# craftsangjae/instance-segmentation-road-project

Measured on AMD Instinct MI355X. Metric: images/sec at 1024x1024 (MaskLab inference hot path, full forward), higher is better.
Workload: dtype f32; 1 GPU; resnext50_full_b8_1024; per_gpu_batch=8, global_batch=8, height=1024, width=1024, parallelism=dp1, hipgraph=False, inputs=resident in HBM, weights=random init (cls logits x8 so NMS / mask head run at full load)

## Files before the change

### include/masklab_hip.h

```cpp
#ifndef MASKLAB_HIP_H
#define MASKLAB_HIP_H

#include <stdint.h>

#ifdef __cplusplus
extern "C" {
#endif

#define ML_OK 0
#define ML_E_BADARG (-1)
#define ML_E_LAUNCH (-2)
#define ML_E_NOGPU  (-3)

enum { ML_ACT_NONE = 0, ML_ACT_RELU = 1, ML_ACT_RELU6 = 2, ML_ACT_SIGMOID = 3 };
enum { ML_MATH_F32 = 0, ML_MATH_F16 = 1, ML_MATH_F16S = 2, ML_MATH_F32X3 = 3 };

#define ML_ABI_VERSION 7
int ml_version(void);
const char *ml_last_error(void);
int ml_device_check(void);

typedef struct ml_conv2d_desc {
    const float *in;
    const float *wgt;
// ... 185 lines not shown
    const void *residual;
    const float *w1, *b1;
    const float *w2, *b2;
    void *out;
    int32_t B, HW, C, Hd;
} ml_se_bottleneck_desc;
int64_t ml_se_bottleneck_workspace_bytes(int32_t B, int32_t HW, int32_t C);
int ml_se_bottleneck_f32(const ml_se_bottleneck_desc *desc, void *workspace, int64_t workspace_bytes, void *stream);
int ml_se_bottleneck_f16(const ml_se_bottleneck_desc *desc, void *workspace, int64_t workspace_bytes, void *stream);

int ml_conv1x1_dual_f32(const float *a, const float *x, const float *wgt, const float *bias, float *out,
                        int32_t B, int32_t H, int32_t W, int32_t Ka, int32_t Kx, int32_t N, int32_t stride, void *stream);
int ml_conv1x1_dual_f16(const void *a, const void *x, const void *wgt, const float *bias, void *out,
                        int32_t B, int32_t H, int32_t W, int32_t Ka, int32_t Kx, int32_t N, int32_t stride, void *stream);

int ml_restore_boxes_f32(const float *loc, const int32_t *priors, float *boxes,
                         int32_t B, int32_t A, void *stream);

int64_t ml_detection_workspace_bytes(int32_t B, int32_t A, int32_t C, int32_t max_out);
int ml_detection_proposal_f32(const float *cls_pred, const float *boxes, float *proposed,
                              int32_t *counts, int32_t *kept, float *gather_payload,
                              int32_t B, int32_t A, int32_t C,
                              float min_confidence, float nms_iou, float post_iou, int32_t max_out,
                              void *workspace, void *stream);

int ml_mask_distribute_i32(const float *rows, int32_t row_stride, int32_t has_k,
                           float *kvals , int32_t *level_slots,
                           int32_t *level_counts, int32_t *level_max, int32_t B, int32_t cap,
                           int32_t max_k, float base_size, void *stream);

// ... 215 lines not shown
```

### instance-segmentation-road-project_amd/csrc/conv1x1_pipe.hip

```cpp
#include <type_traits>
#include "common.h"

namespace {

constexpr int BM = 128, BN = 128;
constexpr int ROWB = 128;
constexpr int BUFB = (BM + BN) * ROWB;
constexpr int SCR_LD = 36;
constexpr int SCRB = 16 * SCR_LD * 4;
constexpr int pipe_lds_bytes(int nstage) { return nstage * BUFB + 4 * SCRB; }
constexpr int PIPE_MAX_NBG = 8;

struct f32x3_t { float v; };

typedef int i32x4 __attribute__((ext_vector_type(4)));
typedef unsigned u32x4 __attribute__((ext_vector_type(4)));

struct PipeArgs {
    const void *in, *wgt, *res;
    const float *bias;
    void *out;
    long long M;
    int K, N;
    int in_cs, in_coff, out_cs, out_coff;
    int panels, NB, grid;
    int units, gshift, NBG;
    int xcd_map;
    float lo, hi;
};

__device__ __forceinline__ void lds_dma16(__amdgpu_buffer_rsrc_t rsrc, char *dst, int voff, int soff) {
#if defined(__HIP_DEVICE_COMPILE__)
    __builtin_amdgcn_raw_ptr_buffer_load_lds(rsrc, (__attribute__((address_space(3))) void *)dst, 16, voff, soff, 0, 0);
#endif
}
__device__ __forceinline__ void buf_store16(f32x4 v, __amdgpu_buffer_rsrc_t rsrc, int voff, int soff) {
#if defined(__HIP_DEVICE_COMPILE__)
    __builtin_amdgcn_raw_buffer_store_b128(__builtin_bit_cast(u32x4, v), rsrc, voff, soff, 0);
#endif
}

__device__ __forceinline__ unsigned records_left(long long off, long long total) {
    const unsigned long long left = (unsigned long long)(total - off);
    const unsigned hi = (unsigned)(left >> 32), lo = (unsigned)left;
    return (hi & 0x80000000u) ? 0u : (hi ? 0xffffffffu : lo);
// ... 79 lines not shown
            v1[c] = __builtin_amdgcn_fmed3f(v1[c], S.lo, S.hi);
        }
    }
    if constexpr (F32) {
        buf_store16(v0, ro, S.t_voff[qn], S.rowoff[(qm * 2 + hs) * 2 + 0]);
        buf_store16(v1, ro, S.t_voff[qn], S.rowoff[(qm * 2 + hs) * 2 + 1]);
    } else {
        const f16x8 o = {(_Float16)v0[0], (_Float16)v0[1], (_Float16)v0[2], (_Float16)v0[3],
                         (_Float16)v1[0], (_Float16)v1[1], (_Float16)v1[2], (_Float16)v1[3]};
        buf_store16(__builtin_bit_cast(f32x4, o), ro, S.t_voff[qn], S.rowoff[(qm * 2 + hs) * 2]);
    }
}

template <class T, bool FIRST, bool HAS_RES, int NB4, bool CLAMP>
__device__ __forceinline__ void pipe_chunk(f32x16 (&cur)[2][2], f32x16 (&oth)[2][2], const PipeState &S, const char *rd,
                                           char *wr, char *scratch, __amdgpu_buffer_rsrc_t ra_nx,
                                           __amdgpu_buffer_rsrc_t rb_nx, int soff_nx, __amdgpu_buffer_rsrc_t ro_prev,
                                           const f32x4 (&bias_prev)[2][NB4], i32x4 rr_prev) {
    constexpr bool F32 = std::is_same<T, float>::value;
    constexpr int NSLOT = F32 ? 64 : 16;
    constexpr int UNITS = F32 ? 2 : 1;
    constexpr int LEAD = HAS_RES ? RES_LEAD : 0;
    constexpr int NREG = FIRST ? NPC + LEAD : 0;
    f32x4 ring[RES_LEAD][2];
    f32x4 fa[2][2], fb[2][2];
    auto read_frags = [&](int ks, f32x4 (&a)[2], f32x4 (&b)[2]) {
#pragma unroll
        for (int m = 0; m < 2; ++m)
            a[m] = *reinterpret_cast<const f32x4 *>(rd + S.a_off + m * 32 * ROWB + (((ks * 2 + S.h) ^ S.swz) * 16));
#pragma unroll
        for (int n = 0; n < 2; ++n)
            b[n] = *reinterpret_cast<const f32x4 *>(rd + S.b_off + n * 32 * ROWB + (((ks * 2 + S.h) ^ S.swz) * 16));
// ... 7 lines not shown
        f32x4 (&a)[2] = fa[ks & 1];
        f32x4 (&b)[2] = fb[ks & 1];
        if constexpr (in_ks == (F32 ? 6 : 1) && ks < 3) read_frags(ks + 1, fa[(ks + 1) & 1], fb[(ks + 1) & 1]);
        constexpr bool start = FIRST && ks == 0 && j == 0;
        const f32x16 zero = {0.f, 0.f, 0.f, 0.f, 0.f, 0.f, 0.f, 0.f, 0.f, 0.f, 0.f, 0.f, 0.f, 0.f, 0.f, 0.f};
        if constexpr (F32) {
            if constexpr (start) cur[mi][ni] = __builtin_amdgcn_mfma_f32_32x32x2f32(a[mi][j], b[ni][j], zero, 0, 0, 0);
            else cur[mi][ni] = __builtin_amdgcn_mfma_f32_32x32x2f32(a[mi][j], b[ni][j], cur[mi][ni], 0, 0, 0);
        } else {
            const f16x8 ha = __builtin_bit_cast(f16x8, a[mi]), hb = __builtin_bit_cast(f16x8, b[ni]);
            if constexpr (start) cur[mi][ni] = __builtin_amdgcn_mfma_f32_32x32x16_f16(ha, hb, zero, 0, 0, 0);
            else cur[mi][ni] = __builtin_amdgcn_mfma_f32_32x32x16_f16(ha, hb, cur[mi][ni], 0, 0, 0);
        }
        __builtin_amdgcn_sched_barrier(0);
        if constexpr (idx < 4) {
            lds_dma16(ra_nx, wr + (32 * idx + 8 * S.wave_u) * ROWB, S.a_voff[idx], soff_nx);
        } else if constexpr (idx < 8) {
            lds_dma16(rb_nx, wr + (BM + 32 * (idx - 4) + 8 * S.wave_u) * ROWB, S.b_voff[idx - 4], soff_nx);
        } else if constexpr (FIRST) {
            constexpr int pb = ((idx - 8) * NREG) / (NSLOT - 8), pe = ((idx - 7) * NREG) / (NSLOT - 8);
            static_for<pb, pe>([&](auto pc) {
                constexpr int p = decltype(pc)::value;
                if constexpr (p >= LEAD) {
                    constexpr int q = p - LEAD;
                    if constexpr (HAS_RES) {
                        constexpr int loads_after = ((p < NPC ? p : NPC) - q - 1) * UNITS;
                        constexpr int stores_after = (q - (q >= LEAD ? q - LEAD + 1 : 0)) * UNITS;
                        constexpr int younger = loads_after + stores_after;
                        static_assert(younger >= 0 && younger <= 63, "vmcnt immediate out of range");
                        if constexpr (F32) wait_loaded<younger>(ring[q % RES_LEAD][0], ring[q % RES_LEAD][1]);
                        else wait_loaded<younger>(ring[q % RES_LEAD][0]);
// ... 89 lines not shown
                for (int ni = 0; ni < 2; ++ni) cur[mi][ni] = __builtin_amdgcn_mfma_f32_32x32x16_f16(ah[mi], bh[ni], cur[mi][ni], 0, 0, 0);
#pragma unroll
            for (int mi = 0; mi < 2; ++mi)
#pragma unroll
                for (int ni = 0; ni < 2; ++ni) crx[mi][ni] = __builtin_amdgcn_mfma_f32_32x32x16_f16(ah[mi], bl[ni], crx[mi][ni], 0, 0, 0);
        }
#pragma unroll
        for (int mi = 0; mi < 2; ++mi)
#pragma unroll
            for (int ni = 0; ni < 2; ++ni)
                crx[mi][ni] = __builtin_amdgcn_mfma_f32_32x32x16_f16(al[mi], bh[ni], crx[mi][ni], 0, 0, 0);
        __builtin_amdgcn_sched_barrier(0);
    }
}

template <class T, bool HAS_RES, int NSTAGE, bool CLAMP>
__global__ void __launch_bounds__(256, NSTAGE == 2 ? 2 : 1)
conv1x1_pipe_kernel(const PipeArgs A) {
    constexpr bool X3 = std::is_same<T, f32x3_t>::value;
    constexpr bool F32 = !std::is_same<T, _Float16>::value;
    constexpr int ES = sizeof(T);
    constexpr int KC = ROWB / ES;
    constexpr int NB4 = F32 ? 1 : 2;
    extern __shared__ __align__(16) char lds[];
    const int tid = threadIdx.x, lane = tid & 63, wave = tid >> 6;
    const int wm = wave >> 1, wn = wave & 1;
    const int r = lane & 31, h = lane >> 5;
    const int ld_row = tid >> 3;
    const int ld_g = (tid & 7) ^ ((ld_row >> 1) & 7);

    PipeState S;
    S.h = h;
    S.swz = (r >> 1) & 7;
    S.a_off = (wm * 64 + r) * ROWB;
    S.b_off = BM * ROWB + (wn * 64 + r) * ROWB;
    S.wave_u = __builtin_amdgcn_readfirstlane(wave);
    S.lo = A.lo;
    S.hi = A.hi;
#pragma unroll
    for (int i = 0; i < 4; ++i) {
        S.a_voff[i] = ((ld_row + 32 * i) * A.in_cs + A.in_coff) * ES + ld_g * 16;
        S.b_voff[i] = (ld_row + 32 * i) * A.K * ES + ld_g * 16;
    }
    const int t_row = F32 ? (lane >> 3) : (lane >> 2);
    const int t_col = F32 ? (lane & 7) * 4 : (lane & 3) * 8;
#pragma unroll
    for (int ni = 0; ni < 2; ++ni)
        S.t_voff[ni] = ((wm * 64 + t_row) * A.out_cs + A.out_coff + wn * 64 + ni * 32 + t_col) * ES;
#pragma unroll
    for (int mi = 0; mi < 2; ++mi)
#pragma unroll
        for (int hs = 0; hs < 2; ++hs)
#pragma unroll
            for (int i = 0; i < 2; ++i) S.rowoff[(mi * 2 + hs) * 2 + i] = (mi * 32 + hs * 16 + 8 * i) * A.out_cs * ES;
    S.scr_w = (4 * h * SCR_LD + r) * 4;
    S.scr_r = (t_row * SCR_LD + t_col) * 4;

    const int nk = A.K / KC;
    const long long in_total = A.M * (long long)A.in_cs * ES;
    const long long out_total = A.M * (long long)A.out_cs * ES;
    const long long w_total = (long long)A.N * A.K * ES;
    const int gmask = (1 << A.gshift) - 1;
    const int step = A.grid >> A.gshift;
    const int bid = (int)blockIdx.x;
    const int slot = bid >> 3, ppx = step >> 3;
    const int group = A.xcd_map ? (slot & gmask) : (bid & gmask);
    const int panel0 = A.xcd_map ? (bid & 7) * ppx + (slot >> A.gshift) : (bid >> A.gshift);
    auto panel_of = [&](Cursor c) { return c.u; };
    auto res_a = [&](Cursor c) { return rsrc_at(A.in, (long long)panel_of(c) * BM * A.in_cs * ES, c.u < A.panels ? in_total : 0); };
    auto res_b = [&](Cursor c) { return rsrc_at(A.wgt, (long long)c.nt * BN * A.K * ES, c.u < A.panels ? w_total : 0); };
    auto tile_off = [&](Cursor c) { return ((long long)panel_of(c) * BM * A.out_cs + (long long)c.nt * BN) * ES; };
    auto res_o = [&](Cursor c) { return rsrc_at(A.out, tile_off(c), c.u < A.panels ? out_total : 0); };
    auto res_words = [&](Cursor c) { return rsrc_words(A.res, tile_off(c), (HAS_RES && c.u < A.panels) ? out_total : 0); };
    const int nt0 = group * A.NBG;
    auto advance = [&](Cursor c) {
        Cursor n = c;
        if (n.nt + 1 < nt0 + A.NBG) { ++n.nt; } else { n.u += step; n.nt = nt0; }
        return n;
    };
    char *scratch = lds + NSTAGE * BUFB + S.wave_u * SCRB;
    float *lds_bias = reinterpret_cast<float *>(lds + NSTAGE * BUFB + 4 * SCRB);
    for (int i = tid; i < A.NBG * BN; i += 256) lds_bias[i] = A.bias ? A.bias[nt0 * BN + i] : 0.f;
    __syncthreads();
    auto bias_at = [&](Cursor c) { return lds_bias + (c.u < A.panels ? c.nt - nt0 : 0) * BN + wn * 64 + t_col; };
// ... 10 lines not shown
    if (cur.u >= A.panels) return;
    Cursor nx = cur;
    int kc_nx = 0;

    f32x16 accA[2][2], accB[2][2];
    f32x4 bias_cur[2][NB4], bias_prev[2][NB4];
#pragma unroll
    for (int ni = 0; ni < 2; ++ni)
#pragma unroll
        for (int k = 0; k < NB4; ++k) bias_prev[ni][k] = f32x4{0.f, 0.f, 0.f, 0.f};
    load_bias(cur, bias_cur);
#pragma unroll
    for (int st = 0; st < NSTAGE - 1; ++st) {
        const __amdgpu_buffer_rsrc_t ra = res_a(nx), rb = res_b(nx);
        const int soff = kc_nx * ROWB;
#pragma unroll
        for (int i = 0; i < 4; ++i) lds_dma16(ra, lds + st * BUFB + (32 * i + 8 * S.wave_u) * ROWB, S.a_voff[i], soff);
#pragma unroll
        for (int i = 0; i < 4; ++i) lds_dma16(rb, lds + st * BUFB + (BM + 32 * i + 8 * S.wave_u) * ROWB, S.b_voff[i], soff);
        ++kc_nx;
        if (kc_nx == nk) { kc_nx = 0; nx = advance(nx); }
    }
    asm volatile("s_waitcnt vmcnt(%0)" ::"n"(8 * (NSTAGE - 2)) : "memory");
    __builtin_amdgcn_s_barrier();

    Cursor prev = {A.panels, 0};
    int buf = 0;
    auto run_tile_x3 = [&](f32x16 (&acc)[2][2], f32x16 (&crx)[2][2]) -> bool {
        const Cursor next = advance(cur);
        const bool has_next = next.u < A.panels;
// ... 19 lines not shown
        prev = cur;
        cur = next;
        return has_next;
    };
    auto run_tile = [&](f32x16 (&acc)[2][2], f32x16 (&oth)[2][2]) -> bool {
        const Cursor next = advance(cur);
        const bool has_next = next.u < A.panels;
        const __amdgpu_buffer_rsrc_t ro_prev = res_o(prev);
        const i32x4 rr_prev = res_words(prev);
        for (int kc = 0; kc < nk; ++kc) {
            const __amdgpu_buffer_rsrc_t ra_nx = res_a(nx), rb_nx = res_b(nx);
            const int soff_nx = kc_nx * ROWB;
            const char *rd = lds + buf * BUFB;
            char *wr = lds + (buf == 0 ? NSTAGE - 1 : buf - 1) * BUFB;
            const bool first = kc == 0;
            if (first) pipe_chunk<T, true, HAS_RES, NB4, CLAMP>(acc, oth, S, rd, wr, scratch, ra_nx, rb_nx, soff_nx, ro_prev, bias_prev, rr_prev);
            else pipe_chunk<T, false, HAS_RES, NB4, CLAMP>(acc, oth, S, rd, wr, scratch, ra_nx, rb_nx, soff_nx, ro_prev, bias_prev, rr_prev);
            ++kc_nx;
            if (kc_nx == nk) { kc_nx = 0; nx = advance(nx); }
            buf = buf + 1 == NSTAGE ? 0 : buf + 1;
            if (kc <= NSTAGE - 2) asm volatile("s_waitcnt vmcnt(%0)" ::"n"(8 * (NSTAGE - 2) + (F32 ? 16 : 8)) : "memory");
            else asm volatile("s_waitcnt vmcnt(%0)" ::"n"(8 * (NSTAGE - 2)) : "memory");
            __builtin_amdgcn_s_barrier();
        }
        prev = cur;
#pragma unroll
        for (int ni = 0; ni < 2; ++ni)
#pragma unroll
            for (int k = 0; k < NB4; ++k) bias_prev[ni][k] = bias_cur[ni][k];
        cur = next;
        if (has_next) load_bias(cur, bias_cur);
        return has_next;
// ... 16 lines not shown
            }
            finish_piece<T, q, HAS_RES, NB4, CLAMP>(acc, S, scratch, ro, bias_prev, r0, r1);
        });
    };
    if constexpr (X3) {
        while (run_tile_x3(accA, accB)) {}
        x3_finish<HAS_RES, CLAMP>(accA, accB, S, scratch, res_o(prev), bias_at(prev), res_words(prev));
    } else {
        for (;;) {
            if (!run_tile(accA, accB)) { drain(accA); break; }
            if (!run_tile(accB, accA)) { drain(accB); break; }
        }
    }
}

template <class T, bool HAS_RES, int NSTAGE, bool CLAMP>
int launch_pipe(const PipeArgs &A, hipStream_t s) {
    auto kern = conv1x1_pipe_kernel<T, HAS_RES, NSTAGE, CLAMP>;
    static std::atomic<unsigned long long> ok{0};
    if (int rc = ml_ensure_dynamic_lds(reinterpret_cast<const void *>(kern), pipe_lds_bytes(NSTAGE) + 4 * PIPE_MAX_NBG * BN, ok,
                                       "conv1x1_pipe"))
        return rc;
    hipLaunchKernelGGL(kern, dim3(A.grid), dim3(256), pipe_lds_bytes(NSTAGE) + 4 * A.NBG * BN, s, A);
    ML_CHECK_LAUNCH("conv1x1_pipe");
    return ML_OK;
}

}

int ml_conv1x1_pipe_eligible(const ml_conv2d_desc &d) {
    const bool f16s = d.math == ML_MATH_F16S, x3 = d.math == ML_MATH_F32X3;
    const int kc = f16s ? 64 : 32;
    const bool shape_ok = d.KH == 1 && d.KW == 1 && d.stride == 1 && d.dil == 1 && d.pad_t == 0 && d.pad_l == 0 &&
                          d.cpp_shift == 30 && d.group_cin_step == 0 && d.shuffle2x2 == 0 && d.out_bstride == 0 &&
                          (d.math == ML_MATH_F32 || f16s || x3) && d.Ho == d.H && d.Wo == d.W;
    if (!shape_ok || d.live || d.gn_partials) return 0;
    if (f16s && !d.out_f16) return 0;
    if (!f16s && d.out_f16) return 0;
    if (d.span % kc != 0 || d.cout % 128 != 0 || d.n_pad != d.cout) return 0;
    if (!f16s && d.span != d.span_pad) return 0;
// ... 7 lines not shown
    int nbg = d.cout / BN;
    for (int g = 1; g < 8 && nbg > PIPE_MAX_NBG && nbg % 2 == 0 && (1 << g) <= ml_resident_blocks(2); ++g) nbg /= 2;
    return nbg <= PIPE_MAX_NBG;
}

int ml_conv1x1_pipe_try(const ml_conv2d_desc &d, hipStream_t s, int *eligible) {
    *eligible = 0;
    if (!ml_conv1x1_pipe_eligible(d)) return ML_OK;
    const long long M = (long long)d.B * d.H * d.W;
    PipeArgs A;
    A.in = d.in; A.wgt = d.wgt; A.bias = d.bias; A.res = d.residual; A.out = d.out;
    A.M = M; A.K = d.span; A.N = d.cout;
    A.in_cs = d.in_cstride; A.in_coff = d.in_coff; A.out_cs = d.out_cstride; A.out_coff = d.out_coff;
    A.panels = (int)((M + BM - 1) / BM);
    A.NB = d.cout / BN;
    const int resident = ml_resident_blocks(2);
    double eff_of[8] = {0, 0, 0, 0, 0, 0, 0, 0}, best_eff = -1.0;
    int n_g = 0;
    for (int g = 0; g < 8 && (A.NB >> g) >= 1 && (A.NB % (1 << g)) == 0; ++g) {
        n_g = g + 1;
        if ((A.NB >> g) > PIPE_MAX_NBG || (1 << g) > resident) continue;
        const long long units = (long long)A.panels << g;
        const long long grid = units < resident ? units : resident / (1 << g) * (1 << g);
        const long long rounds = (units + grid - 1) / grid;
        eff_of[g] = (double)units / (double)(rounds * resident);
        if (eff_of[g] > best_eff) best_eff = eff_of[g];
    }
    if (best_eff <= 0.0) return ML_OK;
    int best = -1, best_map = 0;
    for (int g = n_g - 1; g > 0 && best < 0; --g) {
        if (eff_of[g] <= 0.0 || eff_of[g] < best_eff - 0.02) continue;
        const long long units = (long long)A.panels << g;
        const long long grid = units < resident ? units : resident / (1 << g) * (1 << g);
        if (grid % (8ll << g) == 0) { best = g; best_map = 1; }
    }
    for (int g = 0; g < n_g && best < 0; ++g)
        if (eff_of[g] > 0.0 && eff_of[g] >= best_eff - 0.02) best = g;
    A.gshift = best;
    A.xcd_map = best_map;
    A.NBG = A.NB >> A.gshift;
    A.units = A.panels << A.gshift;
    A.grid = A.units < resident ? A.units : resident / (1 << A.gshift) * (1 << A.gshift);
    const bool clamp = d.act != ML_ACT_NONE;
    A.lo = 0.f;
    A.hi = d.act == ML_ACT_RELU6 ? 6.f : 3.402823466e38f;
    int rc;
    if (d.math == ML_MATH_F16S) {
        if (clamp) rc = d.residual ? launch_pipe<_Float16, true, 2, true>(A, s) : launch_pipe<_Float16, false, 2, true>(A, s);
        else rc = d.residual ? launch_pipe<_Float16, true, 2, false>(A, s) : launch_pipe<_Float16, false, 2, false>(A, s);
    } else if (d.math == ML_MATH_F32X3) {
        if (clamp) rc = d.residual ? launch_pipe<f32x3_t, true, 2, true>(A, s) : launch_pipe<f32x3_t, false, 2, true>(A, s);
        else rc = d.residual ? launch_pipe<f32x3_t, true, 2, false>(A, s) : launch_pipe<f32x3_t, false, 2, false>(A, s);
    } else {
        if (clamp) rc = d.residual ? launch_pipe<float, true, 2, true>(A, s) : launch_pipe<float, false, 2, true>(A, s);
        else rc = d.residual ? launch_pipe<float, true, 2, false>(A, s) : launch_pipe<float, false, 2, false>(A, s);
    }
    if (rc != ML_OK) return rc;
    *eligible = 1;
    return ML_OK;
}
```

### instance-segmentation-road-project_amd/masklab_hip/_lib.py

```python
import ctypes as C
import os

_HERE = os.path.dirname(os.path.abspath(__file__))
LIB_PATH = os.path.join(_HERE, "libmasklab_hip.so")

ABI_VERSION = 7
ACT_NONE, ACT_RELU, ACT_RELU6, ACT_SIGMOID = 0, 1, 2, 3
ACT_BY_NAME = {None: ACT_NONE, "linear": ACT_NONE, "relu": ACT_RELU, "relu6": ACT_RELU6,
               "sigmoid": ACT_SIGMOID}


class ConvDesc(C.Structure):
    _fields_ = [
        ("in_", C.c_void_p), ("wgt", C.c_void_p), ("bias", C.c_void_p),
        ("residual", C.c_void_p), ("out", C.c_void_p),
        ("B", C.c_int32), ("H", C.c_int32), ("W", C.c_int32),
        ("in_cstride", C.c_int32), ("in_coff", C.c_int32),
        ("span", C.c_int32), ("span_pad", C.c_int32), ("cpp_shift", C.c_int32),
        ("Ho", C.c_int32), ("Wo", C.c_int32),
        ("KH", C.c_int32), ("KW", C.c_int32), ("stride", C.c_int32), ("dil", C.c_int32),
        ("pad_t", C.c_int32), ("pad_l", C.c_int32),
        ("cout", C.c_int32), ("n_pad", C.c_int32),
        ("out_cstride", C.c_int32), ("out_coff", C.c_int32),
        ("res_cstride", C.c_int32), ("res_coff", C.c_int32),
# ... 111 lines not shown
    "ml_groupnorm_chunk_stats_f32": (C.c_int, [_vp, _vp, _i32, _i64, _i32, _i32, _vp, _vp]),
    "ml_groupnorm_grad_multi_f32": (C.c_int, [C.POINTER(GnGradDesc), _i32, _vp, _i64, _vp]),
    "ml_resize_bilinear_ac_f32": (C.c_int, [_vp, _vp, _vp] + [_i32] * 12 + [_vp]),
    "ml_global_mean_f32": (C.c_int, [_vp, _vp, _i32, _i32, _i32, _vp]),
    "ml_scale_channels_f32": (C.c_int, [_vp, _vp, _i32, _i32, _i32, _vp]),
    "ml_squeeze_excite_workspace_bytes": (_i64, [_i32, _i32, _i32]),
    "ml_squeeze_excite_f32": (C.c_int, [C.POINTER(SeDesc), _i32, _vp, _i64, _vp]),
    "ml_squeeze_excite_f16": (C.c_int, [C.POINTER(SeDesc), _i32, _vp, _i64, _vp]),
    "ml_se_residual_workspace_bytes": (_i64, [_i32, _i32, _i32]),
    "ml_se_residual_f32": (C.c_int, [C.POINTER(SeResidualDesc), _vp, _i64, _vp]),
    "ml_se_bottleneck_workspace_bytes": (_i64, [_i32, _i32, _i32]),
    "ml_se_bottleneck_f32": (C.c_int, [C.POINTER(SeBottleneckDesc), _vp, _i64, _vp]),
    "ml_se_bottleneck_f16": (C.c_int, [C.POINTER(SeBottleneckDesc), _vp, _i64, _vp]),
    "ml_conv1x1_dual_f32": (C.c_int, [_vp] * 5 + [_i32] * 7 + [_vp]),
    "ml_conv1x1_dual_f16": (C.c_int, [_vp] * 5 + [_i32] * 7 + [_vp]),
    "ml_restore_boxes_f32": (C.c_int, [_vp, _vp, _vp, _i32, _i32, _vp]),
    "ml_detection_workspace_bytes": (_i64, [_i32, _i32, _i32, _i32]),
    "ml_detection_proposal_f32": (C.c_int, [_vp, _vp, _vp, _vp, _vp, _vp, _i32, _i32, _i32, _f32, _f32, _f32, _i32, _vp, _vp]),
    "ml_mask_distribute_i32": (C.c_int, [_vp, _i32, _i32, _vp, _vp, _vp, _vp, _i32, _i32, _i32, _f32, _vp]),
    "ml_roi_crop_resize_f32": (C.c_int, [_vp, _vp, _i32, _i32, _vp, _vp, _vp, _vp] + [_i32] * 10 + [_f32, _f32, _i32, _i32, _vp, _vp]),
    "ml_mold_levels_f32": (C.c_int, [_vp, _vp, _i32, _i32, _i32, _i64, C.POINTER(C.c_int32), _vp]),
    "ml_mold_levels_dev_f32": (C.c_int, [_vp, _vp, _i32, _i32, _i32, _i64, _vp, _vp]),
    "ml_add_f32": (C.c_int, [_vp, _vp, _i64, _vp]),
    "ml_add_f16": (C.c_int, [_vp, _vp, _i64, _vp]),
    "ml_fill_f32": (C.c_int, [_vp, _f32, _i64, _vp]),
    "ml_resize_image_ac": (C.c_int, [_vp, _i32, _vp, _vp, _f32] + [_i32] * 6 + [_vp]),
    "ml_trim_instances_f32": (C.c_int, [_vp] * 5 + [_i32] * 5 + [_vp]),
    "ml_upsample_boxes_i32": (C.c_int, [_vp, _vp, _i64, _f32, _f32, _vp]),
    "ml_threshold_i32": (C.c_int, [_vp, _vp, _f32, _i64, _vp]),
    "ml_semantic_smoothing_f32": (C.c_int, [_vp, _vp, _vp] + [_i32] * 4 + [_vp, _vp, _vp]),
# ... 98 lines not shown
```

### instance-segmentation-road-project_amd/masklab_hip/backbone/body.py

```python
import numpy as np

from .. import ops
from ..keras_like import Layer, WeightSpec

STAGE_TAPS = ("C2", "C3", "C4", "C5")


def bn_data_specs():
    return {
        "bn_data/beta": WeightSpec((3,), "normal", stddev=0.1),
        "bn_data/moving_mean": WeightSpec((3,), "uniform", low=100.0, high=130.0),
        "bn_data/moving_variance": WeightSpec((3,), "uniform", low=3000.0, high=5000.0),
    }


def input_affine(weights, eps):
    mean = np.asarray(weights["bn_data/moving_mean"], np.float64)
    div = np.sqrt(np.asarray(weights["bn_data/moving_variance"], np.float64) + eps)
    return mean.astype(np.float32), div.astype(np.float32), np.asarray(weights["bn_data/beta"], np.float32)


class BatchNorm(Layer):

    def __init__(self, channels, eps, gamma_range=(0.5, 1.5), **kwargs):
# ... 30 lines not shown
        self.add_weight("conv2/kernel", (1, 1, self.hidden, self.channels), "he_normal")
        self.add_weight("conv2/bias", (self.channels,), "normal", stddev=0.1)
        self.built = True
        self.w1 = None

    def _load_own(self, weights, device):
        import torch
        C, Hd = self.channels, self.hidden
        up = lambda a: torch.from_numpy(np.ascontiguousarray(a, np.float32)).to(device)
        self.w1 = up(self._get(weights, "conv1/kernel").reshape(C, Hd))
        self.b1 = up(self._get(weights, "conv1/bias"))
        self.w2 = up(self._get(weights, "conv2/kernel").reshape(Hd, C))
        self.b2 = up(self._get(weights, "conv2/bias"))


class ResidualBody(Layer):
    INPUT_BN_EPS = None
    trailing = ()

    def units(self):
        return [u for st in self.stages for u in st]

    def build(self, input_shape):
        s = self.stem.build(input_shape)
        taps = {"C1": s}
        H, W = s[1], s[2]
        s = (s[0], None if H is None else (H + 2 - 3) // 2 + 1, None if W is None else (W + 2 - 3) // 2 + 1, s[3])
        taps.update(self.stage_shapes(s))
        self.built = True
        return taps
# ... 40 lines not shown
```

### instance-segmentation-road-project_amd/masklab_hip/backbone/resnet50.py

```python
from .. import ops
from ..keras_like import Conv2D
from .body import ResidualBody

BN_EPS = 1e-3
STAGES = ((2, "abc", (64, 64, 256), 1), (3, "abcd", (128, 128, 512), 2), (4, "abcdef", (256, 256, 1024), 2),
          (5, "abc", (512, 512, 2048), 2))


class _DualPack:

    def __init__(self, conv_a, conv_x):
        self.conv_a, self.conv_x, self.dev = conv_a, conv_x, None

    def weight_specs(self):
        return {}

    def load_weights(self, weights, device):
        ka, ba = self.conv_a.folded(weights)
        kx, bx = self.conv_x.folded(weights)
        self.dev = ops.DeviceDualConv(ka, ba, kx, bx, device, dc_a=self.conv_a.dev, dc_x=self.conv_x.dev)


class _Block:

    def __init__(self, filters, stage, block, stride, shortcut):
        conv, bnn = f"res{stage}{block}_branch", f"bn{stage}{block}_branch"
        rng = {"1": (0.5, 1.0), "2a": (0.5, 1.5), "2b": (0.5, 1.5), "2c": (0.1, 0.3)}
        kw = lambda s: dict(fold_bn=(bnn + s, BN_EPS, True, rng[s]), name=conv + s, kernel_initializer="he_normal",
                            bias_initializer="normal")
        f1, f2, f3 = filters
        self.stride = stride
        self.conv2a = Conv2D(f1, 1, strides=stride, activation='relu', **kw("2a"))
        self.conv2b = Conv2D(f2, 3, padding='same', activation='relu', **kw("2b"))
        self.conv2c = Conv2D(f3, 1, activation='relu', **kw("2c"))
        self.shortcut = Conv2D(f3, 1, strides=stride, **kw("1")) if shortcut else None
# ... 30 lines not shown
```

### instance-segmentation-road-project_amd/masklab_hip/backbone/resnext.py

```python
from ..keras_like import Conv2D, GroupedConv2D
from .body import ResidualBody

BN_EPS = 1.001e-5


class _Block:
    def __init__(self, filters, stride, conv_shortcut, name, groups=32):
        rng = {0: (0.5, 1.0), 1: (0.5, 1.5), 2: (0.5, 1.5), 3: (0.1, 0.3)}
        bn = lambda s: (f"{name}_{s}_bn", BN_EPS, True, rng[s])
        he = dict(kernel_initializer="he_normal")
        self.shortcut = None
        if conv_shortcut:
            self.shortcut = Conv2D((64 // groups) * filters, 1, strides=stride, use_bias=False, fold_bn=bn(0),
                                   name=f"{name}_0_conv", **he)
        self.conv1 = Conv2D(filters, 1, use_bias=False, fold_bn=bn(1), activation='relu',
                            name=f"{name}_1_conv", **he)
        self.conv2 = GroupedConv2D(filters, groups, strides=stride, padding=((1, 1), (1, 1)), fold_bn=bn(2),
                                   activation='relu', name=f"{name}_2_conv")
        self.conv3 = Conv2D((64 // groups) * filters, 1, use_bias=False, fold_bn=bn(3), activation='relu',
                            name=f"{name}_3_conv", **he)

    def layers(self):
        return [l for l in (self.shortcut, self.conv1, self.conv2, self.conv3) if l is not None]

    def build(self, shape):
        sc = self.shortcut.build(shape) if self.shortcut is not None else shape
        s = self.conv1.build(shape)
        s = self.conv2.build(s)
        s = self.conv3.build(s)
        assert tuple(s[1:]) == tuple(sc[1:]) or None in s, (s, sc)
        return s

    def __call__(self, x):
        sc = self.shortcut(x) if self.shortcut is not None else x
        y = self.conv1(x)
        y = self.conv2(y)
        return self.conv3(y, residual=sc)


class ResNeXt50(ResidualBody):
    STAGES = (("conv2", 128, 3, 1), ("conv3", 256, 4, 2), ("conv4", 512, 6, 2), ("conv5", 1024, 3, 2))

    def __init__(self, **kwargs):
        super().__init__(name=kwargs.pop("name", "resnext50_body"), **kwargs)
        self.stem = Conv2D(64, 7, strides=2, padding=((3, 3), (3, 3)), use_bias=False,
                           fold_bn=("conv1_bn", BN_EPS, True), activation='relu', image_input=True,
                           kernel_initializer="he_normal", name="conv1_conv")
        self.stages = []
# ... 6 lines not shown
```

### instance-segmentation-road-project_amd/masklab_hip/ops.py

```python
import ctypes as C
import threading

import numpy as np
import torch

from . import _lib
from .packing import PackedConv, pack_winograd, resolve_padding

import weakref

_ws_cache = {}
_ws_retired = []
_graph_owners = weakref.WeakSet()


def graph_owner_registered(model):
    _graph_owners.add(model)


def graph_owner_released(model):
    _graph_owners.discard(model)
    if not len(_graph_owners):
        _ws_retired.clear()

# ... 919 lines not shown
    with _Prof("conv1x1_dual_h" if half else "conv1x1_dual", 2.0 * M * packed.N * (packed.Ka + Kx),
               es * (M * (packed.Ka + Kx) + M * packed.N + w.numel()),
               f"M={M} N={packed.N} Ka={packed.Ka} Kx={Kx} s{stride_b} HxW={H}x{W}") as prof:
        status = fn(_ptr(a), _ptr(x), _ptr(w), _ptr(packed.bias), _ptr(out), B, H, W, packed.Ka, Kx, packed.N, stride_b,
                    _stream())
        if status == -1:
            prof.on = False
        else:
            _lib.check(status, "ml_conv1x1_dual")
    if status == -1:
        sc = conv2d(x, packed.dc_x, stride=stride_b, padding="valid")
        return conv2d(a, packed.dc_a, padding="valid", act=_lib.ACT_RELU, residual=sc)
    return out


def restore_boxes(loc_pred, priors_i32):
    lib = _lib.load()
    _require_dev(loc_pred, "loc_pred")
    B, A, _ = loc_pred.shape
    boxes = torch.empty((B, A, 4), dtype=torch.float32, device=loc_pred.device)
    _lib.check(lib.ml_restore_boxes_f32(_ptr(loc_pred), _ptr(priors_i32), _ptr(boxes), B, A, _stream()),
               "ml_restore_boxes_f32")
    return boxes


def detection_proposal(cls_pred, boxes, min_confidence, nms_iou, post_iou, max_out, want_kept=False,
                       want_payload=False):
    lib = _lib.load()
    _require_dev(cls_pred, "cls_pred")
    _require_dev(boxes, "boxes")
# ... 1271 lines not shown
```

Baseline: 434.1 images/sec.

## Fuse ResNeXt projection shortcut and conv3 into one pipelined dual-source conv1x1

```diff
diff --git a/include/masklab_hip.h b/include/masklab_hip.h
--- a/include/masklab_hip.h
+++ b/include/masklab_hip.h
@@ -223,6 +223,9 @@
 int ml_conv1x1_dual_f16(const void *a, const void *x, const void *wgt, const float *bias, void *out,
                         int32_t B, int32_t H, int32_t W, int32_t Ka, int32_t Kx, int32_t N, int32_t stride, void *stream);
 
+int ml_conv1x1_pipe_dual_f32(const float *a, const float *x, const float *wgt, const float *bias, float *out,
+                             int32_t B, int32_t H, int32_t W, int32_t Ka, int32_t Kx, int32_t N, int32_t stride, void *stream);
+
 int ml_restore_boxes_f32(const float *loc, const int32_t *priors, float *boxes,
                          int32_t B, int32_t A, void *stream);
 
diff --git a/instance-segmentation-road-project_amd/csrc/conv1x1_pipe.hip b/instance-segmentation-road-project_amd/csrc/conv1x1_pipe.hip
--- a/instance-segmentation-road-project_amd/csrc/conv1x1_pipe.hip
+++ b/instance-segmentation-road-project_amd/csrc/conv1x1_pipe.hip
@@ -29,6 +29,15 @@
     float lo, hi;
 };
 
+struct PipeDualArgs : PipeArgs {
+    const void *x;
+    int Ka, x_cs;
+    int H, W, stride, wshift;
+    int ppi, ppr, rows_pp;
+    unsigned ppi_magic, ppr_magic;
+    long long x_total;
+};
+
 __device__ __forceinline__ void lds_dma16(__amdgpu_buffer_rsrc_t rsrc, char *dst, int voff, int soff) {
 #if defined(__HIP_DEVICE_COMPILE__)
     __builtin_amdgcn_raw_ptr_buffer_load_lds(rsrc, (__attribute__((address_space(3))) void *)dst, 16, voff, soff, 0, 0);
@@ -138,8 +147,8 @@
 
 template <class T, bool FIRST, bool HAS_RES, int NB4, bool CLAMP>
 __device__ __forceinline__ void pipe_chunk(f32x16 (&cur)[2][2], f32x16 (&oth)[2][2], const PipeState &S, const char *rd,
-                                           char *wr, char *scratch, __amdgpu_buffer_rsrc_t ra_nx,
-                                           __amdgpu_buffer_rsrc_t rb_nx, int soff_nx, __amdgpu_buffer_rsrc_t ro_prev,
+                                           char *wr, char *scratch, __amdgpu_buffer_rsrc_t ra_nx, const int (&a_voff)[4],
+                                           int soff_a, __amdgpu_buffer_rsrc_t rb_nx, int soff_nx, __amdgpu_buffer_rsrc_t ro_prev,
                                            const f32x4 (&bias_prev)[2][NB4], i32x4 rr_prev) {
     constexpr bool F32 = std::is_same<T, float>::value;
     constexpr int NSLOT = F32 ? 64 : 16;
@@ -177,7 +186,7 @@
         }
         __builtin_amdgcn_sched_barrier(0);
         if constexpr (idx < 4) {
-            lds_dma16(ra_nx, wr + (32 * idx + 8 * S.wave_u) * ROWB, S.a_voff[idx], soff_nx);
+            lds_dma16(ra_nx, wr + (32 * idx + 8 * S.wave_u) * ROWB, a_voff[idx], soff_a);
         } else if constexpr (idx < 8) {
             lds_dma16(rb_nx, wr + (BM + 32 * (idx - 4) + 8 * S.wave_u) * ROWB, S.b_voff[idx - 4], soff_nx);
         } else if constexpr (FIRST) {
@@ -297,9 +306,10 @@
     }
 }
 
-template <class T, bool HAS_RES, int NSTAGE, bool CLAMP>
+template <class T, bool HAS_RES, int NSTAGE, bool CLAMP, bool DUAL = false>
 __global__ void __launch_bounds__(256, NSTAGE == 2 ? 2 : 1)
-conv1x1_pipe_kernel(const PipeArgs A) {
+conv1x1_pipe_kernel(const std::conditional_t<DUAL, PipeDualArgs, PipeArgs> A) {
+    static_assert(!DUAL || (std::is_same<T, float>::value && !HAS_RES), "the second source: fp32, no residual");
     constexpr bool X3 = std::is_same<T, f32x3_t>::value;
     constexpr bool F32 = !std::is_same<T, _Float16>::value;
     constexpr int ES = sizeof(T);
@@ -320,10 +330,15 @@
     S.wave_u = __builtin_amdgcn_readfirstlane(wave);
     S.lo = A.lo;
     S.hi = A.hi;
+    int x_voff[4] = {0, 0, 0, 0};
 #pragma unroll
     for (int i = 0; i < 4; ++i) {
         S.a_voff[i] = ((ld_row + 32 * i) * A.in_cs + A.in_coff) * ES + ld_g * 16;
         S.b_voff[i] = (ld_row + 32 * i) * A.K * ES + ld_g * 16;
+        if constexpr (DUAL) {
+            const int row = ld_row + 32 * i;
+            x_voff[i] = ((row >> A.wshift) * A.W + (row & ((1 << A.wshift) - 1))) * A.stride * A.x_cs * ES + ld_g * 16;
+        }
     }
     const int t_row = F32 ? (lane >> 3) : (lane >> 2);
     const int t_col = F32 ? (lane & 7) * 4 : (lane & 3) * 8;
@@ -351,6 +366,21 @@
     const int panel0 = A.xcd_map ? (bid & 7) * ppx + (slot >> A.gshift) : (bid >> A.gshift);
     auto panel_of = [&](Cursor c) { return c.u; };
     auto res_a = [&](Cursor c) { return rsrc_at(A.in, (long long)panel_of(c) * BM * A.in_cs * ES, c.u < A.panels ? in_total : 0); };
+    int nkA = 0;
+    if constexpr (DUAL) nkA = A.Ka / KC;
+    auto res_x = [&](Cursor c) {
+        if constexpr (DUAL) {
+            const unsigned p = (unsigned)c.u;
+            const unsigned b = (unsigned)(((unsigned long long)p * A.ppi_magic) >> 31), q = p - b * A.ppi;
+            const unsigned i = (unsigned)(((unsigned long long)q * A.ppr_magic) >> 31), jp = q - i * A.ppr;
+            const long long pix = ((long long)b * A.H + (long long)(i * A.rows_pp) * A.stride) * A.W + (long long)jp * BM * A.stride;
+            return rsrc_at(A.x, pix * A.x_cs * ES, c.u < A.panels ? A.x_total : 0);
+        } else {
+            return res_a(c);
+        }
+    };
+    (void)res_x;
+    (void)x_voff;
     auto res_b = [&](Cursor c) { return rsrc_at(A.wgt, (long long)c.nt * BN * A.K * ES, c.u < A.panels ? w_total : 0); };
     auto tile_off = [&](Cursor c) { return ((long long)panel_of(c) * BM * A.out_cs + (long long)c.nt * BN) * ES; };
     auto res_o = [&](Cursor c) { return rsrc_at(A.out, tile_off(c), c.u < A.panels ? out_total : 0); };
@@ -391,6 +421,7 @@
     for (int st = 0; st < NSTAGE - 1; ++st) {
         const __amdgpu_buffer_rsrc_t ra = res_a(nx), rb = res_b(nx);
         const int soff = kc_nx * ROWB;
+        static_assert(!DUAL || NSTAGE == 2, "the prologue stages chunk 0 only, which is the first source's");
 #pragma unroll
         for (int i = 0; i < 4; ++i) lds_dma16(ra, lds + st * BUFB + (32 * i + 8 * S.wave_u) * ROWB, S.a_voff[i], soff);
 #pragma unroll
@@ -440,8 +471,22 @@
             const char *rd = lds + buf * BUFB;
             char *wr = lds + (buf == 0 ? NSTAGE - 1 : buf - 1) * BUFB;
             const bool first = kc == 0;
-            if (first) pipe_chunk<T, true, HAS_RES, NB4, CLAMP>(acc, oth, S, rd, wr, scratch, ra_nx, rb_nx, soff_nx, ro_prev, bias_prev, rr_prev);
-            else pipe_chunk<T, false, HAS_RES, NB4, CLAMP>(acc, oth, S, rd, wr, scratch, ra_nx, rb_nx, soff_nx, ro_prev, bias_prev, rr_prev);
+            if constexpr (DUAL) {
+                const bool second = kc_nx >= nkA;
+                const __amdgpu_buffer_rsrc_t rs_nx = second ? res_x(nx) : ra_nx;
+                const int soff_s = second ? soff_nx - nkA * ROWB : soff_nx;
+                int s_voff[4];
+#pragma unroll
+                for (int i = 0; i < 4; ++i) {
+                    const int xv = x_voff[i], av = S.a_voff[i];
+                    s_voff[i] = second ? xv : av;
+                }
+                if (first) pipe_chunk<T, true, HAS_RES, NB4, CLAMP>(acc, oth, S, rd, wr, scratch, rs_nx, s_voff, soff_s, rb_nx, soff_nx, ro_prev, bias_prev, rr_prev);
+                else pipe_chunk<T, false, HAS_RES, NB4, CLAMP>(acc, oth, S, rd, wr, scratch, rs_nx, s_voff, soff_s, rb_nx, soff_nx, ro_prev, bias_prev, rr_prev);
+            } else {
+                if (first) pipe_chunk<T, true, HAS_RES, NB4, CLAMP>(acc, oth, S, rd, wr, scratch, ra_nx, S.a_voff, soff_nx, rb_nx, soff_nx, ro_prev, bias_prev, rr_prev);
+                else pipe_chunk<T, false, HAS_RES, NB4, CLAMP>(acc, oth, S, rd, wr, scratch, ra_nx, S.a_voff, soff_nx, rb_nx, soff_nx, ro_prev, bias_prev, rr_prev);
+            }
             ++kc_nx;
             if (kc_nx == nk) { kc_nx = 0; nx = advance(nx); }
             buf = buf + 1 == NSTAGE ? 0 : buf + 1;
@@ -488,9 +533,9 @@
     }
 }
 
-template <class T, bool HAS_RES, int NSTAGE, bool CLAMP>
-int launch_pipe(const PipeArgs &A, hipStream_t s) {
-    auto kern = conv1x1_pipe_kernel<T, HAS_RES, NSTAGE, CLAMP>;
+template <class T, bool HAS_RES, int NSTAGE, bool CLAMP, bool DUAL = false>
+int launch_pipe(const std::conditional_t<DUAL, PipeDualArgs, PipeArgs> &A, hipStream_t s) {
+    auto kern = conv1x1_pipe_kernel<T, HAS_RES, NSTAGE, CLAMP, DUAL>;
     static std::atomic<unsigned long long> ok{0};
     if (int rc = ml_ensure_dynamic_lds(reinterpret_cast<const void *>(kern), pipe_lds_bytes(NSTAGE) + 4 * PIPE_MAX_NBG * BN, ok,
                                        "conv1x1_pipe"))
@@ -498,6 +543,37 @@
     hipLaunchKernelGGL(kern, dim3(A.grid), dim3(256), pipe_lds_bytes(NSTAGE) + 4 * A.NBG * BN, s, A);
     ML_CHECK_LAUNCH("conv1x1_pipe");
     return ML_OK;
+}
+
+bool plan_pipe(PipeArgs &A) {
+    const int resident = ml_resident_blocks(2);
+    double eff_of[8] = {0, 0, 0, 0, 0, 0, 0, 0}, best_eff = -1.0;
+    int n_g = 0;
+    for (int g = 0; g < 8 && (A.NB >> g) >= 1 && (A.NB % (1 << g)) == 0; ++g) {
+        n_g = g + 1;
+        if ((A.NB >> g) > PIPE_MAX_NBG || (1 << g) > resident) continue;
+        const long long units = (long long)A.panels << g;
+        const long long grid = units < resident ? units : resident / (1 << g) * (1 << g);
+        const long long rounds = (units + grid - 1) / grid;
+        eff_of[g] = (double)units / (double)(rounds * resident);
+        if (eff_of[g] > best_eff) best_eff = eff_of[g];
+    }
+    if (best_eff <= 0.0) return false;
+    int best = -1, best_map = 0;
+    for (int g = n_g - 1; g > 0 && best < 0; --g) {
+        if (eff_of[g] <= 0.0 || eff_of[g] < best_eff - 0.02) continue;
+        const long long units = (long long)A.panels << g;
+        const long long grid = units < resident ? units : resident / (1 << g) * (1 << g);
+        if (grid % (8ll << g) == 0) { best = g; best_map = 1; }
+    }
+    for (int g = 0; g < n_g && best < 0; ++g)
+        if (eff_of[g] > 0.0 && eff_of[g] >= best_eff - 0.02) best = g;
+    A.gshift = best;
+    A.xcd_map = best_map;
+    A.NBG = A.NB >> A.gshift;
+    A.units = A.panels << A.gshift;
+    A.grid = A.units < resident ? A.units : resident / (1 << A.gshift) * (1 << A.gshift);
+    return true;
 }
 
 }
@@ -535,33 +611,7 @@
     A.in_cs = d.in_cstride; A.in_coff = d.in_coff; A.out_cs = d.out_cstride; A.out_coff = d.out_coff;
     A.panels = (int)((M + BM - 1) / BM);
     A.NB = d.cout / BN;
-    const int resident = ml_resident_blocks(2);
-    double eff_of[8] = {0, 0, 0, 0, 0, 0, 0, 0}, best_eff = -1.0;
-    int n_g = 0;
-    for (int g = 0; g < 8 && (A.NB >> g) >= 1 && (A.NB % (1 << g)) == 0; ++g) {
-        n_g = g + 1;
-        if ((A.NB >> g) > PIPE_MAX_NBG || (1 << g) > resident) continue;
-        const long long units = (long long)A.panels << g;
-        const long long grid = units < resident ? units : resident / (1 << g) * (1 << g);
-        const long long rounds = (units + grid - 1) / grid;
-        eff_of[g] = (double)units / (double)(rounds * resident);
-        if (eff_of[g] > best_eff) best_eff = eff_of[g];
-    }
-    if (best_eff <= 0.0) return ML_OK;
-    int best = -1, best_map = 0;
-    for (int g = n_g - 1; g > 0 && best < 0; --g) {
-        if (eff_of[g] <= 0.0 || eff_of[g] < best_eff - 0.02) continue;
-        const long long units = (long long)A.panels << g;
-        const long long grid = units < resident ? units : resident / (1 << g) * (1 << g);
-        if (grid % (8ll << g) == 0) { best = g; best_map = 1; }
-    }
-    for (int g = 0; g < n_g && best < 0; ++g)
-        if (eff_of[g] > 0.0 && eff_of[g] >= best_eff - 0.02) best = g;
-    A.gshift = best;
-    A.xcd_map = best_map;
-    A.NBG = A.NB >> A.gshift;
-    A.units = A.panels << A.gshift;
-    A.grid = A.units < resident ? A.units : resident / (1 << A.gshift) * (1 << A.gshift);
+    if (!plan_pipe(A)) return ML_OK;
     const bool clamp = d.act != ML_ACT_NONE;
     A.lo = 0.f;
     A.hi = d.act == ML_ACT_RELU6 ? 6.f : 3.402823466e38f;
@@ -580,3 +630,55 @@
     *eligible = 1;
     return ML_OK;
 }
+
+#ifndef PIPE_DUAL_MAX_K
+#define PIPE_DUAL_MAX_K 192
+#endif
+static bool pipe_dual_preferred(int Ka, int Kx, int N) {
+    (void)N;
+    return Ka + Kx <= PIPE_DUAL_MAX_K;
+}
+
+extern "C" int ml_conv1x1_pipe_dual_f32(const float *a, const float *x, const float *wgt, const float *bias, float *out,
+                                        int32_t B, int32_t H, int32_t W, int32_t Ka, int32_t Kx, int32_t N, int32_t stride,
+                                        void *stream) {
+    const char *what = "conv1x1_pipe_dual_f32";
+    constexpr long long LIM = 1ll << 31;
+    ML_REQUIRE(a && x && wgt && bias && out, "%s: a, x, wgt, bias and out are required", what);
+    ML_REQUIRE(B > 0 && H > 0 && W > 0, "%s: B, H and W must be positive", what);
+    ML_REQUIRE(stride == 1 || stride == 2, "%s: stride = %d, must be 1 or 2", what, stride);
+    ML_REQUIRE(Ka > 0 && Kx > 0 && Ka % 32 == 0 && Kx % 32 == 0, "%s: Ka = %d and Kx = %d must be positive multiples of 32", what, Ka, Kx);
+    ML_REQUIRE(N > 0 && N % BN == 0, "%s: N = %d must be a positive multiple of %d", what, N, BN);
+    ML_REQUIRE(ml_aligned16(a) && ml_aligned16(x) && ml_aligned16(wgt) && ml_aligned16(bias) && ml_aligned16(out),
+               "%s: a, x, wgt, bias and out must be 16-byte aligned", what);
+    const long long Ho = (H - 1) / stride + 1, Wo = (W - 1) / stride + 1, HoWo = Ho * Wo;
+    ML_REQUIRE(HoWo % BM == 0 && (Wo % BM == 0 || BM % Wo == 0),
+               "%s: %lld x %lld output pixels per image: Ho Wo must be a multiple of %d and Wo a multiple or a divisor of it", what,
+               Ho, Wo, BM);
+    ML_REQUIRE(pipe_dual_preferred(Ka, Kx, N), "%s: Ka + Kx = %d runs as two launches (above %d)", what, Ka + Kx, PIPE_DUAL_MAX_K);
+    PipeDualArgs A;
+    A.ppi = (int)(HoWo / BM);
+    A.ppr = Wo % BM == 0 ? (int)(Wo / BM) : 1;
+    A.rows_pp = Wo % BM == 0 ? 1 : (int)(BM / Wo);
+    A.wshift = 7;
+    if (Wo < BM) for (A.wshift = 0; (1ll << A.wshift) < Wo; ++A.wshift) {}
+    const long long panels = (long long)B * A.ppi, M = panels * BM;
+    const int resident = ml_resident_blocks(2);
+    const long long x_reach = ((long long)(A.rows_pp - 1) * W + (Wo < BM ? Wo : BM)) * stride * Kx * 4;
+    ML_REQUIRE((long long)BM * Ka * 4 < LIM && (long long)(BM + 32) * N * 4 < LIM && x_reach < LIM && (long long)N * (Ka + Kx) * 4 < LIM * 2,
+               "%s: a row, pixel or weight offset passes 32 bits", what);
+    ML_REQUIRE((panels + resident) * (A.ppi > A.ppr ? A.ppi : A.ppr) < LIM, "%s: too many panels (%lld)", what, panels);
+    A.ppi_magic = (unsigned)((LIM + A.ppi - 1) / A.ppi);
+    A.ppr_magic = (unsigned)((LIM + A.ppr - 1) / A.ppr);
+    A.in = a; A.x = x; A.wgt = wgt; A.bias = bias; A.res = nullptr; A.out = out;
+    A.M = M; A.K = Ka + Kx; A.N = N; A.Ka = Ka; A.x_cs = Kx;
+    A.in_cs = Ka; A.in_coff = 0; A.out_cs = N; A.out_coff = 0;
+    A.H = H; A.W = W; A.stride = stride;
+    A.x_total = (long long)B * H * W * Kx * 4;
+    A.panels = (int)panels;
+    A.NB = N / BN;
+    ML_REQUIRE(plan_pipe(A), "%s: N = %d: no split of its %d tiles fits a block", what, N, A.NB);
+    A.lo = 0.f;
+    A.hi = 3.402823466e38f;
+    return launch_pipe<float, false, 2, true, true>(A, (hipStream_t)stream);
+}
diff --git a/instance-segmentation-road-project_amd/masklab_hip/_lib.py b/instance-segmentation-road-project_amd/masklab_hip/_lib.py
--- a/instance-segmentation-road-project_amd/masklab_hip/_lib.py
+++ b/instance-segmentation-road-project_amd/masklab_hip/_lib.py
@@ -149,6 +149,7 @@
     "ml_se_bottleneck_f16": (C.c_int, [C.POINTER(SeBottleneckDesc), _vp, _i64, _vp]),
     "ml_conv1x1_dual_f32": (C.c_int, [_vp] * 5 + [_i32] * 7 + [_vp]),
     "ml_conv1x1_dual_f16": (C.c_int, [_vp] * 5 + [_i32] * 7 + [_vp]),
+    "ml_conv1x1_pipe_dual_f32": (C.c_int, [_vp] * 5 + [_i32] * 7 + [_vp]),
     "ml_restore_boxes_f32": (C.c_int, [_vp, _vp, _vp, _i32, _i32, _vp]),
     "ml_detection_workspace_bytes": (_i64, [_i32, _i32, _i32, _i32]),
     "ml_detection_proposal_f32": (C.c_int, [_vp, _vp, _vp, _vp, _vp, _vp, _i32, _i32, _i32, _f32, _f32, _f32, _i32, _vp, _vp]),
diff --git a/instance-segmentation-road-project_amd/masklab_hip/backbone/body.py b/instance-segmentation-road-project_amd/masklab_hip/backbone/body.py
--- a/instance-segmentation-road-project_amd/masklab_hip/backbone/body.py
+++ b/instance-segmentation-road-project_amd/masklab_hip/backbone/body.py
@@ -68,6 +68,20 @@
         self.b2 = up(self._get(weights, "conv2/bias"))
 
 
+class _DualPack:
+
+    def __init__(self, conv_a, conv_x):
+        self.conv_a, self.conv_x, self.dev = conv_a, conv_x, None
+
+    def weight_specs(self):
+        return {}
+
+    def load_weights(self, weights, device):
+        ka, ba = self.conv_a.folded(weights)
+        kx, bx = self.conv_x.folded(weights)
+        self.dev = ops.DeviceDualConv(ka, ba, kx, bx, device, dc_a=self.conv_a.dev, dc_x=self.conv_x.dev)
+
+
 class ResidualBody(Layer):
     INPUT_BN_EPS = None
     trailing = ()
diff --git a/instance-segmentation-road-project_amd/masklab_hip/backbone/resnet50.py b/instance-segmentation-road-project_amd/masklab_hip/backbone/resnet50.py
--- a/instance-segmentation-road-project_amd/masklab_hip/backbone/resnet50.py
+++ b/instance-segmentation-road-project_amd/masklab_hip/backbone/resnet50.py
@@ -1,24 +1,10 @@
 from .. import ops
 from ..keras_like import Conv2D
-from .body import ResidualBody
+from .body import ResidualBody, _DualPack
 
 BN_EPS = 1e-3
 STAGES = ((2, "abc", (64, 64, 256), 1), (3, "abcd", (128, 128, 512), 2), (4, "abcdef", (256, 256, 1024), 2),
           (5, "abc", (512, 512, 2048), 2))
-
-
-class _DualPack:
-
-    def __init__(self, conv_a, conv_x):
-        self.conv_a, self.conv_x, self.dev = conv_a, conv_x, None
-
-    def weight_specs(self):
-        return {}
-
-    def load_weights(self, weights, device):
-        ka, ba = self.conv_a.folded(weights)
-        kx, bx = self.conv_x.folded(weights)
-        self.dev = ops.DeviceDualConv(ka, ba, kx, bx, device, dc_a=self.conv_a.dev, dc_x=self.conv_x.dev)
 
 
 class _Block:
diff --git a/instance-segmentation-road-project_amd/masklab_hip/backbone/resnext.py b/instance-segmentation-road-project_amd/masklab_hip/backbone/resnext.py
--- a/instance-segmentation-road-project_amd/masklab_hip/backbone/resnext.py
+++ b/instance-segmentation-road-project_amd/masklab_hip/backbone/resnext.py
@@ -1,5 +1,6 @@
+from .. import ops
 from ..keras_like import Conv2D, GroupedConv2D
-from .body import ResidualBody
+from .body import ResidualBody, _DualPack
 
 BN_EPS = 1.001e-5
 
@@ -10,6 +11,7 @@
         bn = lambda s: (f"{name}_{s}_bn", BN_EPS, True, rng[s])
         he = dict(kernel_initializer="he_normal")
         self.shortcut = None
+        self.stride = stride
         if conv_shortcut:
             self.shortcut = Conv2D((64 // groups) * filters, 1, strides=stride, use_bias=False, fold_bn=bn(0),
                                    name=f"{name}_0_conv", **he)
@@ -19,9 +21,10 @@
                                    activation='relu', name=f"{name}_2_conv")
         self.conv3 = Conv2D((64 // groups) * filters, 1, use_bias=False, fold_bn=bn(3), activation='relu',
                             name=f"{name}_3_conv", **he)
+        self.dual = _DualPack(self.conv3, self.shortcut) if conv_shortcut else None
 
     def layers(self):
-        return [l for l in (self.shortcut, self.conv1, self.conv2, self.conv3) if l is not None]
+        return [l for l in (self.shortcut, self.conv1, self.conv2, self.conv3, self.dual) if l is not None]
 
     def build(self, shape):
         sc = self.shortcut.build(shape) if self.shortcut is not None else shape
@@ -32,6 +35,8 @@
         return s
 
     def __call__(self, x):
+        if self.dual is not None and ops.resnext_unit_fused():
+            return ops.conv1x1_pipe_dual(self.conv2(self.conv1(x)), x, self.dual.dev, self.stride)
         sc = self.shortcut(x) if self.shortcut is not None else x
         y = self.conv1(x)
         y = self.conv2(y)
diff --git a/instance-segmentation-road-project_amd/masklab_hip/ops.py b/instance-segmentation-road-project_amd/masklab_hip/ops.py
--- a/instance-segmentation-road-project_amd/masklab_hip/ops.py
+++ b/instance-segmentation-road-project_amd/masklab_hip/ops.py
@@ -957,6 +957,50 @@
     return out
 
 
+RESNEXT_UNIT_FUSION = "on"
+
+
+def set_resnext_unit_fusion(mode):
+    global RESNEXT_UNIT_FUSION
+    if mode not in ("on", "off"):
+        raise ValueError(f"ResNeXt unit fusion must be 'on' or 'off', got {mode!r}")
+    RESNEXT_UNIT_FUSION = mode
+
+
+def resnext_unit_fused():
+    return RESNEXT_UNIT_FUSION == "on" and CONV_MATH == "f32"
+
+
+def conv1x1_pipe_dual(a, x, packed: DeviceDualConv, stride_b=1):
+    lib = _lib.load()
+    _require_dev(a, "a")
+    _require_dev(x, "x")
+    if a.dtype != torch.float32 or x.dtype != torch.float32:
+        raise ValueError(f"conv1x1_pipe_dual: a and x must be float32, got {a.dtype} and {x.dtype}")
+    if stride_b not in (1, 2):
+        raise ValueError(f"conv1x1_pipe_dual: stride_b must be 1 or 2, got {stride_b}")
+    B, H, W, Kx = x.shape
+    Ho, Wo = (H - 1) // stride_b + 1, (W - 1) // stride_b + 1
+    if tuple(a.shape) != (B, Ho, Wo, packed.Ka) or Kx != packed.Kx:
+        raise ValueError(f"conv1x1_pipe_dual: a {tuple(a.shape)} / x {tuple(x.shape)} do not match the packed unit "
+                         f"(Ka={packed.Ka}, Kx={packed.Kx}, stride {stride_b})")
+    out = torch.empty((B, Ho, Wo, packed.N), dtype=a.dtype, device=a.device)
+    M = B * Ho * Wo
+    with _Prof("conv1x1_pipe_dual", 2.0 * M * packed.N * (packed.Ka + Kx),
+               4 * (M * (packed.Ka + Kx) + M * packed.N + packed.wgt.numel()),
+               f"M={M} N={packed.N} Ka={packed.Ka} Kx={Kx} s{stride_b} HxW={H}x{W}") as prof:
+        status = lib.ml_conv1x1_pipe_dual_f32(_ptr(a), _ptr(x), _ptr(packed.wgt), _ptr(packed.bias), _ptr(out), B, H, W,
+                                              packed.Ka, Kx, packed.N, stride_b, _stream())
+        if status == -1:
+            prof.on = False
+        else:
+            _lib.check(status, "ml_conv1x1_pipe_dual_f32")
+    if status == -1:
+        sc = conv2d(x, packed.dc_x, stride=stride_b, padding="valid")
+        return conv2d(a, packed.dc_a, padding="valid", act=_lib.ACT_RELU, residual=sc)
+    return out
+
+
 def restore_boxes(loc_pred, priors_i32):
     lib = _lib.load()
     _require_dev(loc_pred, "loc_pred")
```

After: 437.4 images/sec, median of 6. About the same (+0.7%).
